# tomka/mitsuba-renderer

Measured on AMD Instinct MI355X. Metric: Msamples/s, higher is better.
Workload: dtype f32; 1 GPU; C3 1M-tri Cornell: 1024000-tri displaced walls TriMesh + 20480-tri dielectric icosphere + area light, path maxDepth=16 rrDepth=10, 1024x1024, ldsampler 64 spp per GPU (64 per frame, weak scaling), box filter; triangles=1044482, kd_nodes=551229, kd_indices=1101661, parallelism=ImageBlock tiles, morton(tx, ty) % 1 + one RCCL film reduce per frame

## Files before the change

include/mtsgpu.h:

```cpp
#ifndef MTSGPU_H
#define MTSGPU_H

#include <stdint.h>
#include <stddef.h>

#ifdef __cplusplus
extern "C" {
#endif

#define MTSGPU_ABI_VERSION 8

enum {
	MTSGPU_OK = 0,
	MTSGPU_EINVAL = -1,
	MTSGPU_EHIP = -2,
	MTSGPU_ENODEV = -3,
	MTSGPU_ECANCEL = -4,
	MTSGPU_ESTATE = -5
};

enum {
	MTSGPU_BSDF_LAMBERTIAN = 0,
	MTSGPU_BSDF_DIELECTRIC = 1,
	MTSGPU_BSDF_ROUGHMETAL = 2,
// ... 191 lines not shown
int  mtsgpu_bsdf_eval(mtsgpu_ctx *ctx, uint32_t bsdf_type, const float *params, int op, uint32_t n, const float *queries, float *out);
int  mtsgpu_bsdf_eval_table(mtsgpu_ctx *ctx, uint32_t n_bsdfs, const uint32_t *types, const float *params, uint32_t index, int op,
                            uint32_t n, const float *queries, float *out);
int  mtsgpu_sky_configure(const float *block, float *derived);
int  mtsgpu_lum_eval(mtsgpu_ctx *ctx, uint32_t lum_type, const float *block, int op, uint32_t n, const float *queries, float *out);
int  mtsgpu_scene_lum_eval(mtsgpu_ctx *ctx, int op, uint32_t n, const float *queries, float *out);
int  mtsgpu_vertex_color_eval(mtsgpu_ctx *ctx, uint32_t n, const uint32_t *prim, const float *uv, float *out);
int  mtsgpu_bsdf_eval_colored(mtsgpu_ctx *ctx, uint32_t bsdf_type, const float *params, uint32_t slots, const float color[3], int op,
                              uint32_t n, const float *queries, float *out);
int  mtsgpu_uv_texture_eval(mtsgpu_ctx *ctx, const mtsgpu_uv_texture *tex, uint32_t n, const uint32_t *prim, const float *rec, float *out);
int  mtsgpu_bsdf_eval_slots(mtsgpu_ctx *ctx, uint32_t bsdf_type, const float *params, const int32_t slot_source[2], const float color[3],
                            const float *values, int op, uint32_t n, const float *queries, float *out);
int  mtsgpu_shading_frame_eval(mtsgpu_ctx *ctx, uint32_t n, const uint32_t *prim, const float *rec, float *out);
int  mtsgpu_li_samples(mtsgpu_ctx *ctx, const uint32_t *pix_samples, uint32_t n, float *out);
int  mtsgpu_pass_samples(mtsgpu_ctx *ctx, uint32_t first, uint32_t n, float *out);

typedef struct mtsgpu_mesh {
	uint32_t n_verts, n_tris;
	const float    *positions;
	const float    *normals;
	const uint32_t *triangles;
	int32_t face_normals;
	int32_t bsdf;
	int32_t lum;
	int32_t shape_type;
	float   sphere_center[3];
	float   sphere_radius;
	int32_t sphere_inverted;
} mtsgpu_mesh;

// ... 58 lines not shown
```

mitsuba-renderer_amd/__init__.py:

```python
import ctypes as C
import os
import subprocess

import numpy as np

from . import abi, scenes, filmreduce, testmode
from .testmode import write_mfile, analyze

_HERE = os.path.dirname(os.path.abspath(__file__))
LIB_PATH = os.environ.get("MTSGPU_LIB") or os.path.join(_HERE, "libmtsgpu.so")

EXPORTS = [
    "mtsgpu_create", "mtsgpu_destroy", "mtsgpu_last_error", "mtsgpu_abi_version", "mtsgpu_source_hash", "mtsgpu_abi_sizeof", "mtsgpu_set_stream",
    "mtsgpu_upload_scene", "mtsgpu_set_camera", "mtsgpu_set_integrator", "mtsgpu_set_direct_integrator", "mtsgpu_set_sampler",
    "mtsgpu_set_tiles", "mtsgpu_set_rfilter", "mtsgpu_set_film_edges", "mtsgpu_tabulate_filter", "mtsgpu_set_film_buffer", "mtsgpu_set_options", "mtsgpu_render", "mtsgpu_sync",
    "mtsgpu_read_film", "mtsgpu_clear_film", "mtsgpu_get_stats", "mtsgpu_trace_rays", "mtsgpu_ld_tables",
    "mtsgpu_li_samples", "mtsgpu_flatten", "mtsgpu_flat_scene_get", "mtsgpu_flat_scene_free",
    "mtsgpu_flat_scene_kdstats", "mtsgpu_make_camera", "mtsgpu_make_camera_ortho", "mtsgpu_load_serialized", "mtsgpu_loaded_mesh_free",
    "mtsgpu_make_camera_crop", "mtsgpu_hbm_triad", "mtsgpu_sampler_values", "mtsgpu_random_values", "mtsgpu_set_tuning", "mtsgpu_gather_roof",
    "mtsgpu_create_multi", "mtsgpu_group_destroy", "mtsgpu_group_size", "mtsgpu_group_ctx", "mtsgpu_group_last_error",
    "mtsgpu_group_upload_scene", "mtsgpu_group_set_camera", "mtsgpu_group_set_integrator", "mtsgpu_group_set_sampler",
    "mtsgpu_group_set_rfilter", "mtsgpu_group_render", "mtsgpu_group_last_reduce_kind", "mtsgpu_group_rccl_ranks", "mtsgpu_group_reduce_note", "mtsgpu_bsdf_eval", "mtsgpu_bsdf_eval_table", "mtsgpu_replay_roof", "mtsgpu_group_set_tuning",
    "mtsgpu_sky_configure", "mtsgpu_lum_eval", "mtsgpu_scene_lum_eval", "mtsgpu_pass_samples",
    "mtsgpu_set_film_statistics", "mtsgpu_read_film_statistics", "mtsgpu_film_statistics_form", "mtsgpu_group_set_film_statistics",
    "mtsgpu_set_vertex_colors", "mtsgpu_group_set_vertex_colors", "mtsgpu_flat_scene_set_mesh_colors", "mtsgpu_flat_scene_vertex_colors",
    "mtsgpu_flat_scene_shape_has_colors", "mtsgpu_loaded_mesh_colors", "mtsgpu_vertex_color_eval", "mtsgpu_bsdf_eval_colored",
    "mtsgpu_set_uv_textures", "mtsgpu_group_set_uv_textures", "mtsgpu_flat_scene_set_mesh_texcoords", "mtsgpu_flat_scene_vertex_texcoords",
    "mtsgpu_flat_scene_shape_has_texcoords", "mtsgpu_loaded_mesh_texcoords", "mtsgpu_uv_texture_eval", "mtsgpu_bsdf_eval_slots",
    "mtsgpu_flatten_tangents", "mtsgpu_flat_scene_vertex_tangents", "mtsgpu_flat_scene_shape_has_tangents", "mtsgpu_upload_scene_tangents",
    "mtsgpu_group_upload_scene_tangents", "mtsgpu_shading_frame_eval",
]


class MtsGpuError(RuntimeError):
    pass


def load_serialized(path, shape_index=0, bsdf=-1, lum=-1, name=None):
    h = C.c_void_p(); m = abi.Mesh()
    rc = lib().mtsgpu_load_serialized(os.fsencode(path), int(shape_index), C.byref(h), C.byref(m))
    if rc != 0:
        raise MtsGpuError("mtsgpu_load_serialized: %s" % lib().mtsgpu_last_error(None).decode())
    try:
        pos = abi.np_from(m.positions, (m.n_verts, 3), np.float32)
        tri = abi.np_from(m.triangles, (m.n_tris, 3), np.uint32)
# ... 87 lines not shown
    L.mtsgpu_set_tiles.argtypes = [vp, C.c_int, C.c_int, C.c_int]
    L.mtsgpu_set_film_buffer.argtypes = [vp, vp]
    L.mtsgpu_set_rfilter.argtypes = [vp, C.c_float, C.c_float, f32p]
    L.mtsgpu_set_film_edges.argtypes = [vp, C.c_int]
    L.mtsgpu_tabulate_filter.argtypes = [C.c_int, C.c_float, C.c_float, C.c_float, f32p, f32p]
    L.mtsgpu_set_options.argtypes = [vp, C.c_uint64, C.c_int, C.c_int]
    L.mtsgpu_render.argtypes = [vp, C.POINTER(C.c_int)]
    L.mtsgpu_sync.argtypes = [vp]
    L.mtsgpu_read_film.argtypes = [vp, f32p]
    L.mtsgpu_clear_film.argtypes = [vp]
    L.mtsgpu_get_stats.argtypes = [vp, C.POINTER(abi.Stats)]
    L.mtsgpu_trace_rays.argtypes = [vp, f32p, C.c_uint32, C.c_int, u32p]
    L.mtsgpu_ld_tables.argtypes = [vp, C.c_uint32, f32p, f32p]
    L.mtsgpu_li_samples.argtypes = [vp, u32p, C.c_uint32, f32p]
    L.mtsgpu_pass_samples.argtypes = [vp, C.c_uint32, C.c_uint32, f32p]
    L.mtsgpu_flatten.argtypes = [C.POINTER(abi.SceneDesc), C.POINTER(abi.KdParams), C.POINTER(vp)]
    L.mtsgpu_flat_scene_get.argtypes = [vp]; L.mtsgpu_flat_scene_get.restype = C.POINTER(abi.Scene)
    L.mtsgpu_flat_scene_free.argtypes = [vp]; L.mtsgpu_flat_scene_free.restype = None
    L.mtsgpu_flat_scene_kdstats.argtypes = [vp, C.POINTER(C.c_double)]
    L.mtsgpu_make_camera.argtypes = [f32p, f32p, f32p, C.c_float, C.c_int, C.c_int, C.POINTER(abi.Camera)]
    L.mtsgpu_make_camera_ortho.argtypes = [f32p, f32p, f32p, C.c_float, C.c_float, C.c_int, C.c_int, C.POINTER(abi.Camera)]
    L.mtsgpu_load_serialized.argtypes = [C.c_char_p, C.c_int, C.POINTER(vp), C.POINTER(abi.Mesh)]
    L.mtsgpu_loaded_mesh_free.argtypes = [vp]; L.mtsgpu_loaded_mesh_free.restype = None
    L.mtsgpu_make_camera_crop.argtypes = [f32p, f32p, f32p, C.c_float] + [C.c_int] * 6 + [C.POINTER(abi.Camera)]
    L.mtsgpu_gather_roof.argtypes = [C.c_int, C.c_size_t, C.POINTER(C.c_double)]
    L.mtsgpu_set_tuning.argtypes = [vp, C.c_char_p, C.c_long]
    L.mtsgpu_sampler_values.argtypes = [vp, C.c_uint32, C.c_uint32, C.c_uint32, C.c_int, f32p]
    L.mtsgpu_random_values.argtypes = [vp, C.c_int, C.c_uint64, C.c_uint64, C.c_uint32, C.c_uint32, C.POINTER(C.c_uint64)]
    L.mtsgpu_bsdf_eval.argtypes = [vp, C.c_uint32, f32p, C.c_int, C.c_uint32, f32p, f32p]
    L.mtsgpu_bsdf_eval_table.argtypes = [vp, C.c_uint32, u32p, f32p, C.c_uint32, C.c_int, C.c_uint32, f32p, f32p]
# ... 300 lines not shown

    def sync(self):
        self._chk(lib().mtsgpu_sync(self._ctx), "sync")

    def film(self):
        cam = self.camera.c if hasattr(self.camera, "c") else self.camera
        out = np.zeros((cam.height, cam.width, 5), dtype=np.float32)
        self._chk(lib().mtsgpu_read_film(self._ctx, abi.ptr(out, abi.f32p)), "read_film")
        return out

    def stats(self):
        st = abi.Stats()
        self._chk(lib().mtsgpu_get_stats(self._ctx, C.byref(st)), "get_stats")
        return st.as_dict()

    def set_film_statistics(self, on=True):
        self._chk(lib().mtsgpu_set_film_statistics(self._ctx, int(bool(on))), "set_film_statistics")

    def film_statistics(self):
        cam = self.camera.c if hasattr(self.camera, "c") else self.camera
        var = np.zeros((cam.height, cam.width, 3), dtype=np.float32)
        n = np.zeros((cam.height, cam.width), dtype=np.uint32)
        self._chk(lib().mtsgpu_read_film_statistics(self._ctx, abi.ptr(var, abi.f32p), abi.ptr(n, abi.u32p)), "read_film_statistics")
        return var, n

    def film_statistics_form(self):
        return {0: "lane", 1: "wave"}.get(lib().mtsgpu_film_statistics_form(self._ctx))

    def trace_rays(self, rays, shadow=False):
        r = np.ascontiguousarray(rays, dtype=np.float32).reshape(-1, 8)
# ... 327 lines not shown
```

mitsuba-renderer_amd/csrc/api.cpp:

```cpp
#include "host.h"
#include "kernels.h"
#include "devmath.h"
#include "ctx.h"
#include <algorithm>
#include <cstdarg>
#include <cstdio>
#include <cstring>
#include <cstdlib>
#include <cmath>

using namespace mg;

namespace mg {
thread_local std::string g_lastError;

int fail(mtsgpu_ctx *ctx, int code, const char *fmt, ...) {
	char buf[512];
	va_list ap; va_start(ap, fmt); vsnprintf(buf, sizeof(buf), fmt, ap); va_end(ap);
	g_lastError = buf;
	if (ctx) ctx->error = buf;
	return code;
}
}

// ... 146 lines not shown
	cfg.weight_bsdf = 1 / (float) c->nBsdfSamples; cfg.weight_lum = 1 / (float) c->nLumSamples;
	cfg.frac_bsdf = c->nBsdfSamples / (float) (c->nLumSamples + c->nBsdfSamples);
	cfg.frac_lum = c->nLumSamples / (float) (c->nLumSamples + c->nBsdfSamples);
	cfg.sampler_kind = c->samplerKind;
	cfg.spp = effectiveSpp(c); cfg.ld_depth = c->ldDepth; cfg.seed = c->seed;
	cfg.strat_res = 1; while ((uint32_t) cfg.strat_res * (uint32_t) cfg.strat_res < cfg.spp) ++cfg.strat_res;
	cfg.slot_per_path = slotPerPath ? 1 : 0;
	cfg.ld_scr = c->ldScr; cfg.ld_perm = c->ldPerm; cfg.primes = c->primes;
	if (c->integrator == 1) {
		if (c->nLumSamples > 1) cfg.arr_size[cfg.arr_n++] = (uint32_t) c->nLumSamples;
		if (c->nBsdfSamples > 1) cfg.arr_size[cfg.arr_n++] = (uint32_t) c->nBsdfSamples;
		for (int a = 0; a < cfg.arr_n; ++a) { cfg.arr_off[a] = cfg.arr_total; cfg.arr_total += cfg.spp * cfg.arr_size[a]; }
	}
	cfg.arr_scr = c->arrScr; cfg.arr_perm = c->arrPerm; cfg.arr_pts = c->arrPts;
	cfg.filt_size_x = c->filtSizeX; cfg.filt_size_y = c->filtSizeY; cfg.filt_border = c->filtBorder; cfg.filt_values = c->filtValues;
	return cfg;
}

int ensureSampleArrays(mtsgpu_ctx *c, size_t nSlots, size_t nPaths) {
	if (c->integrator != 1 || (c->nLumSamples <= 1 && c->nBsdfSamples <= 1))
		return 0;
	if (c->samplerKind == MTSGPU_SAMPLER_HALTON || c->samplerKind == MTSGPU_SAMPLER_HAMMERSLEY)
		return fail(c, MTSGPU_EINVAL, "request2DArray() is not supported by QMC samplers! (halton.cpp:102-104, hammersley.cpp:112-114)");
	const uint32_t spp = effectiveSpp(c);
	size_t total = 0; int nArr = 0;
	for (int n : { c->nLumSamples, c->nBsdfSamples })
		if (n > 1) {
			if ((uint64_t) spp * (uint64_t) n > 65536ull)
				return fail(c, MTSGPU_EINVAL, "sampleCount x samples per strategy = %llu exceeds 65536 points per pixel", (unsigned long long) spp * n);
			total += (size_t) spp * n; ++nArr;
// ... 15 lines not shown
hipEvent_t *nextEventPair(mtsgpu_ctx *c, std::vector<std::pair<hipEvent_t, hipEvent_t>> &pool, size_t &used) {
	if (used == pool.size()) {
		hipEvent_t a, b;
		if (hipEventCreate(&a) != hipSuccess || hipEventCreate(&b) != hipSuccess) return nullptr;
		pool.emplace_back(a, b);
	}
	return &pool[used++].first;
}

long tuningOr(const mtsgpu_ctx *c, const char *key, long dflt);
void rayQueues(mtsgpu_ctx *c, const uint32_t *cur, const uint32_t *nxt) {
	const bool on = tuningOr(c, "ray_queues", 1) != 0;
	auto of = [&](const uint32_t *q, int k) -> float4 * { return !on || !q ? nullptr : (q == c->queueA ? c->rayqA[k] : (q == c->queueB ? c->rayqB[k] : nullptr)); };
	c->paths.rq_o = of(cur, 0); c->paths.rq_d = of(cur, 1); c->paths.rqn_o = of(nxt, 0); c->paths.rqn_d = of(nxt, 1);
}
struct RayQueuesOff { mtsgpu_ctx *c; ~RayQueuesOff() { rayQueues(c, nullptr, nullptr); c->q.nee_parked = 0; } };

hipEvent_t *nextTraceEvents(mtsgpu_ctx *c, int cls) {
	hipEvent_t *ev = nextEventPair(c, c->traceEvents, c->traceEvUsed);
	if (ev) {
		if (c->traceEvClass.size() < c->traceEvUsed) c->traceEvClass.resize(c->traceEvUsed);
		c->traceEvClass[c->traceEvUsed - 1] = (unsigned char) cls;
	}
	return ev;
}

int readCounters(mtsgpu_ctx *c) {
	HIPCHK(c, hipMemcpyAsync(c->hostCounters, c->q.counters, kNumCounters * kCounterStride * sizeof(uint32_t), hipMemcpyDeviceToHost, c->stream));
	HIPCHK(c, hipStreamSynchronize(c->stream));
	return 0;
}
// ... 13 lines not shown
		c->stats.trace_launches++;
		int rc = readCounters(c); if (rc) { c->q.force_static = 0; return rc; }
		c->q.force_static = 0;
		bool overflow = false;
		for (int b = 0; b < kNumBins; ++b) {
			uint32_t acc = 0;
			for (int k = 0; k < kBinShards; ++k) {
				views[b].prefix[k] = acc;
				const uint32_t cnt = c->hostCounters[(b * kBinShards + k) * kCounterStride];
				if (cnt > c->q.bin_seg_cap) overflow = true;
				acc += cnt;
			}
			views[b].prefix[kBinShards] = acc;
		}
		if (attempt == 0 && c->tuning.count("test_retry") && c->tuning["test_retry"]) overflow = true;
		if (!overflow) return 0;
		c->stats.bin_overflow_retries++;
	}
	return fail(c, MTSGPU_EHIP, "internal: bin segment overflow with static dealing");
}

int runDirectRounds(mtsgpu_ctx *c, const DConfig &cfg0, uint32_t nPaths, volatile const int *cancel) {
	hipStream_t s = c->stream;
	DConfig cfg = cfg0;
	const size_t counterBytes = kNumCounters * kCounterStride * sizeof(uint32_t);
	auto timedTrace = [&](int mode, bool bin, const uint32_t *queue, uint32_t n, bool coherent) -> int {
		hipEvent_t *ev = c->timeKernels ? nextTraceEvents(c, mode == 1 ? 2 : 0) : nullptr;
		if (ev) HIPCHK(c, hipEventRecord(ev[0], s));
		launch_trace(s, mode, c->countTraversal, bin, c->dsc, c->paths, c->q, queue, n, coherent);
		if (ev) HIPCHK(c, hipEventRecord(ev[1], s));
		HIPCHK(c, hipGetLastError());
// ... 66 lines not shown
	const int chunk = (int) tuningOr(c, "chunk", 8);
	uint32_t *cur = c->queueA, *nxt = c->queueB;
	uint32_t upper = nPaths;
	bool shadowPending = false;
	int b = 0;
	struct Restore {
		mtsgpu_ctx *c; hipStream_t s2; const bool &pending;
		~Restore() {
			if (pending) (void) hipStreamSynchronize(s2);
			c->q.dev_stats = nullptr; c->q.counters = c->counterSets; c->q.spill = c->spillClosest;
		}
	} restore{ c, s2, shadowPending };
	RayQueuesOff rqOff{ c };
	c->q.nee_parked = tuningOr(c, "nee_parked", 1) != 0 ? 1u : 0u;
	if (!c->q.nee_parked) { int rc = ensureNeeQueue(c); if (rc) return rc; }
	auto timed = [&](std::vector<std::pair<hipEvent_t, hipEvent_t>> &pool, size_t &used, hipStream_t s, int which, int cls = -1) -> int {
		if (!c->timeKernels) return 0;
		hipEvent_t *ev = which == 0 ? (cls >= 0 ? nextTraceEvents(c, cls) : nextEventPair(c, pool, used)) : &pool[used - 1].first;
		if (!ev) return fail(c, MTSGPU_EHIP, "hipEventCreate failed");
		HIPCHK(c, hipEventRecord(ev[which], s));
		return 0;
	};
	while (b < limit && upper > 0) {
		if (cancel && *cancel) return fail(c, MTSGPU_ECANCEL, "render cancelled");
		const int end = (int) std::min<long long>((long long) b + chunk, limit);
		for (; b < end; ++b) {
			uint32_t *set = counterSet(c, b), *prev = counterSet(c, b - 1);
			c->q.counters = set; c->q.next = nxt; c->q.spill = c->spillClosest;
			rayQueues(c, cur, nxt);
			int rc = timed(c->traceEvents, c->traceEvUsed, s1, 0, b == 0 ? 1 : 0); if (rc) return rc;
// ... 36 lines not shown
		upper = *hostNext;
	}
	if (shadowPending) {
		HIPCHK(c, hipStreamWaitEvent(s1, c->evShadow[(b - 1) & 1], 0));
		shadowPending = false;
	}
	return 0;
}

int collectDeviceStats(mtsgpu_ctx *c) {
	if (!c->devStatsUsed) return 0;
	c->devStatsUsed = false;
	unsigned long long h[kNumDevStats];
	HIPCHK(c, hipMemcpy(h, c->devStats, sizeof(h), hipMemcpyDeviceToHost));
	c->stats.rays_closest += h[kStatClosest]; c->stats.rays_shadow += h[kStatShadow]; c->stats.trace_launches += h[kStatLaunches];
	if (h[kStatOverflow]) return fail(c, MTSGPU_EHIP, "internal: bin segment overflow in a device-driven frame");
	return 0;
}

int runBounces(mtsgpu_ctx *c, const DConfig &cfg, uint32_t nPaths, volatile const int *cancel) {
	c->q.counters = c->counterSets; c->q.spill = c->spillClosest; c->q.dev_stats = nullptr;
	if (cfg.integrator == 1 && (cfg.n_lum > 1 || cfg.n_bsdf > 1))
		return runDirectRounds(c, cfg, nPaths, cancel);
	{
		const long sf = tuningOr(c, "sync_free", -1);
		if (sf == 1 || (sf < 0 && nPaths <= (8u << 20)))
			return runBouncesDevice(c, cfg, nPaths, cancel);
	}
	uint32_t nQ = nPaths;
	uint32_t *cur = c->queueA, *nxt = c->queueB;
	bool first = true;
	hipStream_t s = c->stream;
	const size_t setBytes = (size_t) kNumCounters * kCounterStride * sizeof(uint32_t);
	RayQueuesOff rqOff{ c };
	c->q.nee_parked = tuningOr(c, "nee_parked", 1) != 0 ? 1u : 0u;
	if (!c->q.nee_parked) { int rc = ensureNeeQueue(c); if (rc) return rc; }
	for (int b = 0; nQ > 0; ++b) {
		if (cancel && *cancel)
			return fail(c, MTSGPU_ECANCEL, "render cancelled");
		c->q.counters = counterSet(c, b); c->q.spill = c->spillClosest;
		HIPCHK(c, hipMemsetAsync(c->q.counters, 0, setBytes, s));
		c->q.next = nxt;
		rayQueues(c, cur, nxt);
		BinView views[kNumBins];
		int rc = traceAndBin(c, cur, nQ, first, views); if (rc) return rc;
		c->stats.rays_closest += nQ;
		hipEvent_t *sev = c->timeKernels ? nextEventPair(c, c->shadeEvents, c->shadeEvUsed) : nullptr;
		if (sev) HIPCHK(c, hipEventRecord(sev[0], s));
		for (int bin = 0; bin < kNumBins; ++bin)
			launch_shade(s, bin, c->dsc, c->paths, cfg, c->q, views[bin], nullptr, 0, nullptr, c->dcol, c->dtex, c->dtan);
		if (sev) HIPCHK(c, hipEventRecord(sev[1], s));
// ... 759 lines not shown
	tabulateFilter(kind, half_size, p0, p1, size_xy, values);
	return 0;
}

int mtsgpu_set_film_buffer(mtsgpu_ctx *c, void *device_ptr) {
	if (!c) return fail(nullptr, MTSGPU_EINVAL, "null context");
	if (c->ownFilm && c->film) (void) hipFree(c->film);
	c->film = (float *) device_ptr; c->ownFilm = false; c->filmPixels = 0;
	return 0;
}

int mtsgpu_set_tuning(mtsgpu_ctx *c, const char *key, long value) {
	if (!c || !key) return fail(c, MTSGPU_EINVAL, "null argument");
	struct Knob { const char *key; long lo, hi; };
	static const Knob knobs[] = { { "refill_min", 1, 64 }, { "desc_min", 1, 64 }, { "leaf_min", 1, 64 }, { "batch", 0, 64 },
	                              { "dyn_div", 0, 1 << 20 }, { "test_retry", 0, 1 }, { "sync_free", -1, 1 }, { "chunk", 1, 1024 }, { "blocks_per_cu", 0, (long) kTraceBlocksPerCuMax }, { "plain_below", 0, 1 << 30 }, { "dyn_min_rounds", 0, 1 << 20 }, { "shade_fused", 0, 1 }, { "ray_queues", 0, 1 }, { "nee_parked", 0, 1 }, { "stats_wave", -1, 1 } };
	for (const Knob &k : knobs)
		if (std::strcmp(k.key, key) == 0) {
			if (value < k.lo || value > k.hi) return fail(c, MTSGPU_EINVAL, "tuning knob %s: %ld outside [%ld, %ld]", key, value, k.lo, k.hi);
			c->tuning[key] = value;
			applyTuning(c);
			return 0;
		}
	return fail(c, MTSGPU_EINVAL, "unknown tuning knob '%s'", key);
}

int mtsgpu_set_options(mtsgpu_ctx *c, uint64_t max_paths, int count_traversal, int time_kernels) {
	if (!c) return fail(nullptr, MTSGPU_EINVAL, "null context");
	c->maxPaths = max_paths; c->countTraversal = count_traversal != 0; c->timeKernels = time_kernels != 0;
	return 0;
}
// ... 96 lines not shown
		for (int t = 0; t < tx * ty; ++t) {
			if (tileMorton((uint32_t) (t % tx), (uint32_t) (t / tx)) % (uint32_t) c->nParts != (uint32_t) c->part) continue;
			const int x0 = off + (t % tx) * bs, y0 = off + (t / tx) * bs;
			TileMeta tm{};
			tm.x0 = x0 + cx; tm.y0 = y0 + cy; tm.w = std::min(bs, off + RW - x0); tm.h = std::min(bs, off + RH - y0);
			tm.slot_base = (uint32_t) pixels.size(); tm.block_index = (uint32_t) tiles.size();
			tm.colour = (uint32_t) (((t % tx) & 1) + 2 * ((t / tx) & 1));
			tiles.push_back(tm);
			for (int y = tm.y0; y < tm.y0 + tm.h; ++y)
				for (int x = tm.x0; x < tm.x0 + tm.w; ++x)
					pixels.push_back((uint32_t) (y - off) * (uint32_t) keyW + (uint32_t) (x - off));
		}
		c->renderKey = key; c->renderListValid = false;
	}
	std::memset(&c->stats, 0, sizeof(c->stats));
	c->traceEvUsed = c->shadeEvUsed = 0;
	if (pixels.empty()) return 0;
	if (!reuse) {
		rc = ensureBuf(c, &c->pixelList, &c->pixelListCap, pixels.size()); if (rc) return rc;
		HIPCHK(c, hipMemcpyAsync(c->pixelList, pixels.data(), pixels.size() * sizeof(uint32_t), hipMemcpyHostToDevice, c->stream));
		HIPCHK(c, hipStreamSynchronize(c->stream));
		c->renderListValid = true;
	}

	const bool wideFilter = c->filtBorder > 0;
	if (wideFilter && 2 * c->filtBorder > bs) return fail(c, MTSGPU_EINVAL, "filter border %d too wide for block size %d", c->filtBorder, bs);
	const uint64_t maxPaths = c->maxPaths ? c->maxPaths : defaultMaxPaths(c);
	size_t slotsPerPass = (size_t) std::max<uint64_t>(1, std::min<uint64_t>(pixels.size(), maxPaths / spp));
	if (wideFilter) slotsPerPass = std::max<size_t>(slotsPerPass, (size_t) bs * bs);
	if ((uint64_t) slotsPerPass * spp > 0x7FFFFFFFull) return fail(c, MTSGPU_EINVAL, "pass too large");
// ... 178 lines not shown
	}
	if (kind == 2) {
		RR_CHK(hipMalloc((void **) &tmp, (size_t) n * 2 * sizeof(float4)));
		launch_gather_strided(s, tmp, c->paths.shq_o, n, stride); launch_gather_strided(s, tmp + n, c->paths.shq_d, n, stride);
		RR_CHK(hipMemcpyAsync(c->paths.shq_o, tmp, (size_t) n * sizeof(float4), hipMemcpyDeviceToDevice, s));
		RR_CHK(hipMemcpyAsync(c->paths.shq_d, tmp + n, (size_t) n * sizeof(float4), hipMemcpyDeviceToDevice, s));
		c->lastPass.shadowMax = 0;
	} else {
		launch_iota_strided(s, c->queueA, n, stride);
		launch_gather_strided(s, c->rayqA[0], c->paths.base + 0, n, stride * kPathSlots);
		launch_gather_strided(s, c->rayqA[1], c->paths.base + 1, n, stride * kPathSlots);
		rayQueues(c, c->queueA, nullptr);
	}
	RayQueuesOff rqOff{ c };
	c->q.nee_parked = mode == 1 ? 1u : 0u;
	const uint32_t *queue = mode == 1 ? c->q.shadow : c->queueA;
	RR_CHK(hipMemsetAsync(recLen, 0, (size_t) n * 4, s));
	RR_CHK(hipMemsetAsync(c->q.trace_counts, 0, kNumTraceCounts * sizeof(unsigned long long), s));
	RR_CHK(hipMemsetAsync(c->q.counters, 0, counterBytes, s));
	c->q.rec = rec; c->q.rec_len = recLen; c->q.rec_cap = cap;
	launch_trace(s, mode, true, bin, c->dsc, c->paths, c->q, queue, n, coherent);
	c->q.rec = c->q.rec_len = nullptr; c->q.rec_cap = 0;
	RR_CHK(hipGetLastError());
	std::vector<uint32_t> len(n);
	RR_CHK(hipMemcpyAsync(len.data(), recLen, (size_t) n * 4, hipMemcpyDeviceToHost, s));
	RR_CHK(hipStreamSynchronize(s));
	unsigned long long cnt[kNumTraceCounts];
	RR_CHK(hipMemcpy(cnt, c->q.trace_counts, sizeof(cnt), hipMemcpyDeviceToHost));
	std::vector<uint32_t> ord(n), first(cap + 2, 0u);
	unsigned long long total = 0, truncated = 0;
// ... 391 lines not shown
		launch_scene_lum_eval(c->stream, c->dsc, op, n, dQ, dOut);
		e = hipGetLastError();
	}
	if (e == hipSuccess) e = hipMemcpyAsync(out, dOut, (size_t) n * 16 * sizeof(float), hipMemcpyDeviceToHost, c->stream);
	if (e == hipSuccess) e = hipStreamSynchronize(c->stream);
	if (dQ) (void) hipFree(dQ);
	if (dOut) (void) hipFree(dOut);
	if (e != hipSuccess) return fail(c, MTSGPU_EHIP, "scene luminaire read-out failed: %s", hipGetErrorString(e));
	return 0;
}

int mtsgpu_li_samples(mtsgpu_ctx *c, const uint32_t *pix_samples, uint32_t n, float *out) {
	int rc = checkReady(c); if (rc) return rc;
	if (!pix_samples || !out) return fail(c, MTSGPU_EINVAL, "null argument");
	std::memset(&c->stats, 0, sizeof(c->stats));
	c->traceEvUsed = c->shadeEvUsed = 0;
	if (n == 0) return 0;
	const uint32_t spp = effectiveSpp(c);
	std::vector<uint32_t> keys(n);
	for (uint32_t i = 0; i < n; ++i) {
		const uint32_t x = pix_samples[3 * (size_t) i], y = pix_samples[3 * (size_t) i + 1], j = pix_samples[3 * (size_t) i + 2];
		if (x >= (uint32_t) c->cam.width || y >= (uint32_t) c->cam.height || j >= spp)
			return fail(c, MTSGPU_EINVAL, "sample %u: pixel or sample index out of range", i);
		keys[i] = (y + (uint32_t) c->cam.crop_offset_y) * (uint32_t) filmWidth(c) + x + (uint32_t) c->cam.crop_offset_x;
	}
	rc = ensurePaths(c, n); if (rc) return rc;
	rc = ensureBuf(c, &c->explicitSamples, &c->explicitCap, 3 * (size_t) n); if (rc) return rc;
	c->renderListValid = false; c->lastPass.valid = false;
	rc = ensureBuf(c, &c->pixelList, &c->pixelListCap, n); if (rc) return rc;
	HIPCHK(c, hipMemcpyAsync(c->explicitSamples, pix_samples, 3 * (size_t) n * sizeof(uint32_t), hipMemcpyHostToDevice, c->stream));
// ... 54 lines not shown
	HIPCHK(c, hipMemcpy2DAsync(misc.data(), 16, rec + 6, pitch, 16, n, hipMemcpyDeviceToHost, c->stream));
	HIPCHK(c, hipStreamSynchronize(c->stream));
	for (size_t i = 0; i < n; ++i) {
		uint32_t flags; int depth;
		std::memcpy(&flags, &Li[4 * i + 3], 4); std::memcpy(&depth, &thr[4 * i + 3], 4);
		float *o = out + 8 * i;
		const float4 L = settled_Li(make_float4(Li[4 * i], Li[4 * i + 1], Li[4 * i + 2], 0.0f),
		                            make_float4(parked[4 * i], parked[4 * i + 1], parked[4 * i + 2], parked[4 * i + 3]));
		o[0] = L.x; o[1] = L.y; o[2] = L.z; o[3] = (flags & F_ALPHA) ? 1.0f : 0.0f;
		o[4] = spos[4 * i]; o[5] = spos[4 * i + 1]; o[6] = (float) depth;
		std::memcpy(&o[7], &misc[4 * i + 3], 4);
	}
	return 0;
}

struct mtsgpu_flat_scene { FlatScene fs; };

int mtsgpu_flatten(const mtsgpu_scene_desc *desc, const mtsgpu_kd_params *kd, mtsgpu_flat_scene **out) {
	if (!desc || !out) return fail(nullptr, MTSGPU_EINVAL, "null argument");
	*out = nullptr;
	try {
		std::unique_ptr<mtsgpu_flat_scene> p(new mtsgpu_flat_scene());
		flattenScene(*desc, kd, p->fs);
		*out = p.release();
	} catch (const std::exception &e) {
		return fail(nullptr, MTSGPU_EINVAL, "%s", e.what());
	}
	return 0;
}

// ... 80 lines not shown
```

mitsuba-renderer_amd/csrc/ctx.h:

```cpp
#pragma once
#include "host.h"
#include "kernels.h"
#include <map>
#include <string>
#include <utility>
#include <vector>

struct mtsgpu_ctx {
	int device = 0;
	uint32_t nCUs = 256;
	hipStream_t stream = nullptr;
	bool ownStream = false;
	hipStream_t stream2 = nullptr;
	hipEvent_t evShade[2] = { nullptr, nullptr }, evShadow[2] = { nullptr, nullptr }, evCount = nullptr;
	std::string error;

	bool haveScene = false;
	mg::DScene dsc{};
	std::vector<void *> sceneAllocs;
	uint32_t nTris = 0;
	struct HostScene {
		uint32_t nVerts = 0;
		std::vector<uint32_t> triIdx, shapeTriOffset, shapeType, bsdfType, lumType;
		std::vector<int32_t> shapeBsdf;
// ... 43 lines not shown
	float4 *primSave = nullptr; size_t primSaveCap = 0;
	float4 *shqNee = nullptr; size_t shqNeeCap = 0;
	uint16_t *primes = nullptr;
	uint32_t *explicitSamples = nullptr; size_t explicitCap = 0;
	uint32_t *hostCounters = nullptr;
	uint32_t *counterSets = nullptr;
	uint32_t *spillClosest = nullptr, *spillShadow = nullptr;
	mg::BinView *viewsDev = nullptr;
	unsigned long long *devStats = nullptr;
	bool devStatsUsed = false;
	uint32_t binMask = 0x1FFu;
	unsigned long long *pathLen = nullptr;
	std::vector<void *> pathAllocs;

	mtsgpu_stats stats{};
	std::vector<std::pair<hipEvent_t, hipEvent_t>> traceEvents, shadeEvents;
	size_t traceEvUsed = 0, shadeEvUsed = 0;
	std::vector<unsigned char> traceEvClass;
	struct LastPass { bool valid = false; mg::DConfig cfg{}; size_t base = 0; uint32_t nSlots = 0, nPaths = 0, shadowMax = 0; } lastPass;
};


namespace mg {
extern thread_local std::string g_lastError;
int fail(mtsgpu_ctx *ctx, int code, const char *fmt, ...);
}

#define HIPCHK(ctx, expr) do { hipError_t e_ = (expr); if (e_ != hipSuccess) \
	return mg::fail(ctx, MTSGPU_EHIP, "%s failed: %s (%s:%d)", #expr, hipGetErrorString(e_), __FILE__, __LINE__); } while (0)
```

mitsuba-renderer_amd/csrc/kernels.h:

```cpp
#pragma once
#include <hip/hip_runtime.h>
#include <stdint.h>

namespace mg {

constexpr int kNumBsdfTypes = 10;
constexpr int kNumBins = kNumBsdfTypes + 1;
#ifndef MG_TRACE_BLOCK
#define MG_TRACE_BLOCK 512
#endif
constexpr int kTraceBlock = MG_TRACE_BLOCK;
static_assert(kTraceBlock % 256 == 0 && kTraceBlock <= 1024, "whole multiples of four waves");
#ifdef MG_TRACE_WGS
constexpr unsigned trace_blocks_per_cu(int) { return MG_TRACE_WGS; }
#else
constexpr unsigned trace_blocks_per_cu(int mode) { return (mode == 0 ? 24u : 32u) / (kTraceBlock / 64); }
#endif
constexpr unsigned trace_waves_per_simd(int mode) { return trace_blocks_per_cu(mode) * (kTraceBlock / 64) / 4; }
constexpr unsigned kTraceBlocksPerCuMax = 2048 / kTraceBlock;
#ifndef MG_STACK_LDS
#define MG_STACK_LDS 10
#endif
#ifndef MG_TOP_PAIRS
#define MG_TOP_PAIRS (MG_TRACE_BLOCK >= 512 ? 1024 : 128)
// ... 13 lines not shown
constexpr int kCounterStride = 32;
constexpr int kBsdfNParams = 16;
constexpr int kBinShards = 16;
constexpr uint32_t kShadeAllBins = ((1u << kNumBins) - 1u) & ~(1u << 9);
constexpr int kNumCounters = kNumBins * kBinShards + 4;
constexpr int kCounterSets = 2;
constexpr int kCntNext = kNumBins * kBinShards, kCntShadow = kCntNext + 1, kCntDynClosest = kCntNext + 2, kCntDynShadow = kCntNext + 3;
constexpr int kNextWord = kCntNext * kCounterStride, kShadowWord = kCntShadow * kCounterStride;
#ifndef MG_SHADE_BLOCK
#define MG_SHADE_BLOCK 1024
#endif
constexpr int kShadeBlock = MG_SHADE_BLOCK;
constexpr int kNumTraceCounts = 16;
enum { kCntPairGlobal = 8, kCntPairLds = 9, kCntNodeGlobal = 10, kCntNodeLds = 11, kCntTail = 12, kCntSpill = 13, kCntHead = 14 };
enum : uint32_t { kReqPair = 1, kReqNode = 2, kReqLeaf = 3, kReqRay = 4, kReqHit = 5, kReqNone = 0xFFFFFFFFu };
enum { kStatClosest = 0, kStatShadow = 1, kStatOverflow = 2, kStatLaunches = 3, kNumDevStats = 4 };

struct DScene {
	const uint2    *nodes;
	const uint4    *leaf_ta;
	const float4   *tri_pos;
	const float4   *tri_nrm;
	const int32_t  *shape_bsdf, *shape_lum;
	const uint32_t *shape_bin;
	const uint32_t *shape_type;
	const float    *shape_params;
	const float    *env_pixels, *env_pdf, *env_cdf;
	uint32_t        env_width, env_height, env_pdf_width, env_pdf_height;
	uint32_t        has_shapes;
	const uint32_t *shape_flags, *shape_tri_offset;
	const uint32_t *bsdf_type;
// ... 95 lines not shown
	uint32_t arr_size[2], arr_off[2], arr_total;
	const uint32_t *arr_scr;
	const uint16_t *arr_perm;
	const float2 *arr_pts;
	int32_t sampler_kind;
	uint32_t spp; int32_t ld_depth;
	int32_t strat_res;
	uint64_t seed;
	int32_t slot_per_path;
	float filt_size_x, filt_size_y;
	int32_t filt_border;
	const float *filt_values;
	const uint32_t *ld_scr;
	const uint16_t *ld_perm;
	const uint16_t *primes;
};

struct DQueues {
	uint32_t *bins_base;
	uint32_t bin_stride;
	uint32_t bin_seg_cap;
	uint4 *bin_hits;
	__host__ __device__ uint32_t *bin(int b) const { return bins_base + (size_t) b * bin_stride; }
	uint32_t *next;
	uint32_t *shadow;
	uint32_t *counters;
	unsigned long long *trace_counts;
	uint32_t *rec, *rec_len;
	uint32_t rec_cap;
	unsigned long long *dev_stats;
	uint32_t *spill;
	uint32_t spill_stride;
	uint32_t desc_min;
	uint32_t leaf_min;
	uint32_t refill_min;
	uint32_t coherent;
	uint32_t n_cus;
	uint32_t force_static;
	uint32_t tune_batch;
	uint32_t tune_dyn_div;
	uint32_t tune_refill;
	uint32_t tune_plain_below;
	uint32_t tune_dyn_min_rounds;
	uint32_t tune_blocks_per_cu;
// ... 109 lines not shown
```

mitsuba-renderer_amd/csrc/shade_path.h:

```cpp
#pragma once
#include "shade_bsdf.h"

namespace mg {

#ifndef MG_SHADE_PACKED
#define MG_SHADE_PACKED 0
#endif
constexpr int kRowStride = MG_SHADE_PACKED ? kPathSlots : kPathSlots + 1;
struct ShadeRow {
	float4 *base; uint32_t x;
	__device__ __forceinline__ float4 &operator[](int k) const { return base[MG_SHADE_PACKED ? ((uint32_t) k ^ x) : (uint32_t) k]; }
};
__device__ __forceinline__ uint32_t shade_row_index(uint32_t lane, uint32_t k) { return lane * kRowStride + (MG_SHADE_PACKED ? (k ^ (lane & 7u)) : k); }

template <int BT, bool ROUNDS, bool SKY, int VCOL, bool TAN = false>
__device__ __forceinline__ void shade_path(const DScene &sc, const DPaths &ps, const DConfig &cfg, const uint32_t id,
                                           const float4 ro, const float4 rd, const uint4 h, const float4 T4, const float4 L4,
                                           const ShadeRow row, bool &continues, bool &wantShadow, V3 &neeV, V3 &shO, V3 &shD, const DColors &col,
                                           const DTextures &tex, const DTangents &tan = DTangents{ nullptr, nullptr }) {
	{
		const int mode = ROUNDS ? cfg.dr_mode : 0;
		const bool skipToNee = ROUNDS && mode == 1 && cfg.dr_index > 0, skipToBsdf = ROUNDS && mode == 2;
		const V3 rayO(ro.x, ro.y, ro.z), rayD(rd.x, rd.y, rd.z);
		const bool valid = h.w != kNoPrim;
		V3 thr(T4.x, T4.y, T4.z), Li(L4.x, L4.y, L4.z);
		int depth = __float_as_int(T4.w);
		uint32_t flags = __float_as_uint(L4.w);
		PathSampler smp;
		uint2 misc_zw;
		{
			const uint4 r = reinterpret_cast<const uint4 &>(row[6]);
			smp.stream = (uint64_t) r.x | ((uint64_t) r.y << 32);
			smp.slot = cfg.slot_per_path ? id : (id / cfg.spp);
			smp.j = r.z;
			misc_zw = make_uint2(r.z, r.w);
			smp.d1 = (flags >> F_D1_SHIFT) & 0xFFu; smp.d2 = (flags >> F_D2_SHIFT) & 0xFFu;
		}
		const bool direct = cfg.integrator == 1;
		Its its;
		if (valid) {
			if (TAN) fill_its_tan(sc, tan, rayO, rayD, __uint_as_float(h.x), h.w, __uint_as_float(h.y), __uint_as_float(h.z), row[0], row[1], row[3], its);
			else fill_its(sc, rayO, rayD, __uint_as_float(h.x), h.w, __uint_as_float(h.y), __uint_as_float(h.z), row[0], row[1], row[3], its);
		}
		const int shapeLum = valid ? sc.shape_lum[its.shape] : -1;

		do {
			if (skipToNee || skipToBsdf) {
			} else if (flags & F_FIRST) {
				flags &= ~F_FIRST;
				if (valid) flags |= F_ALPHA;
				if (!direct && !(depth <= cfg.max_depth || cfg.max_depth < 0))
					break;
			} else {
// ... 5 lines not shown
				V3 lvalue(0, 0, 0), lp(0, 0, 0), ln(0, 0, 0);
				int llum = -1;
				if (valid) {
					if (shapeLum >= 0) {
						const float *LP = sc.lum_params + kLumStride * (size_t) shapeLum;
						lp = its.p; ln = its.geoN; llum = shapeLum;
						lvalue = (dot(-rayD, its.geoN) <= 0) ? V3(0, 0, 0) : V3(LP[0], LP[1], LP[2]);
						hitLuminaire = true;
					}
				} else {
					if (sc.background_lum >= 0) {
						llum = sc.background_lum;
						lvalue = background_le<SKY>(sc, rayD);
						hitLuminaire = true;
					} else {
						if (!direct) depth++;
						break;
					}
				}
				if (hitLuminaire) {
					const float lumPdf = (!(sampledType & T_DELTA)) ? pdf_luminaire(sc, rayO, llum, lp, ln, -rayD) : 0.0f;
					const float weight = direct ? mi_weight(bsdfPdf * cfg.frac_bsdf, lumPdf * cfg.frac_lum) * cfg.weight_bsdf
					                            : mi_weight(bsdfPdf, lumPdf);
					Li.x += thr.x * lvalue.x * bsdfVal.x * weight;
					Li.y += thr.y * lvalue.y * bsdfVal.y * weight;
					Li.z += thr.z * lvalue.z * bsdfVal.z * weight;
				}
				if (!valid || direct)
					break;
				flags &= ~F_EMITTED;
				if (depth >= cfg.rr_depth && !(sampledType & T_TRANSMISSION)) {
					const float approxAlbedo = smin(0.9f, smax(smax(bsdfVal.x, bsdfVal.y), bsdfVal.z));
					if (sampler_next1d(cfg, smp) > approxAlbedo)
						break;
					thr = thr * (1.0f / approxAlbedo);
				}
				thr = thr * bsdfVal;
				depth++;
				if (!(depth <= cfg.max_depth || cfg.max_depth < 0))
					break;
			}

			if (!valid) {
				if (skipToNee || skipToBsdf) break;
				if ((flags & F_EMITTED) && sc.background_lum >= 0) {
					const V3 le = background_le<SKY>(sc, rayD);
					Li.x += thr.x * le.x; Li.y += thr.y * le.y; Li.z += thr.z * le.z;
				}
				break;
			}
			if (BT == kNumBsdfTypes)
				break;
			const int bsdfIdx = sc.shape_bsdf[its.shape];
// ... 86 lines not shown
			const V3 wo(its.shS.x * woL.x + its.shT.x * woL.y + its.shN.x * woL.z,
			            its.shS.y * woL.x + its.shT.y * woL.y + its.shN.y * woL.z,
			            its.shS.z * woL.x + its.shT.z * woL.y + its.shN.z * woL.z);
			const float woDotGeoN = dot(its.geoN, wo);
			if (woDotGeoN * woL.z <= 0 && strict)
				break;
			row[0] = make_float4(its.p.x, its.p.y, its.p.z, kEpsilon);
			row[1] = make_float4(wo.x, wo.y, wo.z, MG_INF);
			row[5] = make_float4(bsdfVal.x, bsdfVal.y, bsdfVal.z, bsdfPdf);
			flags = (flags & 0x00FFFFFFu) | (sampledType << F_ST_SHIFT);
			continues = true;
		} while (false);
		if (!continues) { row[0] = ro; row[1] = rd; }

		flags = (flags & ~((0xFFu << F_D1_SHIFT) | (0xFFu << F_D2_SHIFT))) | (smp.d1 << F_D1_SHIFT) | (smp.d2 << F_D2_SHIFT);
		row[3] = make_float4(thr.x, thr.y, thr.z, __int_as_float(depth));
		row[4] = make_float4(Li.x, Li.y, Li.z, __uint_as_float(flags));
		reinterpret_cast<uint4 &>(row[6]) = make_uint4((uint32_t) (smp.stream & 0xFFFFFFFFull), (uint32_t) (smp.stream >> 32), misc_zw.x, misc_zw.y);
	}

}

#ifndef MG_SHADE_WAVES
#define MG_SHADE_WAVES 0
#endif
#if MG_SHADE_WAVES
#define MG_SHADE_BOUNDS __launch_bounds__(kShadeBlock, MG_SHADE_WAVES)
#else
#define MG_SHADE_BOUNDS __launch_bounds__(kShadeBlock)
#endif
struct ShadeShared {
// ... 193 lines not shown
```

mitsuba-renderer_amd/csrc/trace.hip:

```cpp
#include "kdevice.h"

namespace mg {


__device__ __forceinline__ uint32_t lanes_below(uint64_t mask) {
	return __builtin_amdgcn_mbcnt_hi((uint32_t) (mask >> 32), __builtin_amdgcn_mbcnt_lo((uint32_t) mask, 0u));
}
size_t trace_spill_levels() { return kSpillLevels; }
size_t trace_stack_levels() { return kStackLDS + kSpillLevels; }
uint32_t trace_top_nodes() { return kTopNodes; }

__device__ __forceinline__ const uint4 *leaf_head(const DTraceScene &sc, uint32_t e) { return &sc.leaf_ta[kLeafStride * (size_t) e]; }
__device__ __forceinline__ const uint4 *leaf_tail(const DTraceScene &sc, uint32_t e, uint32_t half) { return &sc.leaf_ta[kLeafStride * (size_t) e + 1 + half]; }

template <int MODE, bool COUNT, bool BIN, bool PARKED>
__device__ __forceinline__ void trace_body(const DTraceScene &sc, const DPaths &ps, const DQueues &q, const TracePlan &plan,
                                           const uint32_t *queue, uint32_t n, const uint32_t first, const uint32_t stride,
                                           uint32_t (*s_stack)[kTraceBlock], uint32_t (*s_mbox)[kTraceBlock], const uint4 *s_top) {
	uint32_t g_pair = 0, l_pair = 0, g_node = 0, l_node = 0, g_tail = 0, g_spill = 0, g_head = 0;
	uint32_t rec_n = 0, rec_slot = 0;
	auto rec_add = [&](uint32_t kind, uint32_t idx) {
		if (COUNT && q.rec) {
			if (rec_n < q.rec_cap) q.rec[(size_t) rec_slot * q.rec_cap + rec_n] = (kind << 29) | idx;
			rec_n++;
// ... 56 lines not shown
				if (base < n) { sup_base = (uint32_t) base; sup_left = (n - sup_base < B) ? n - sup_base : B; }
				else dyn_done = true;
			}
		}
		const uint32_t remaining = sup_left;
		if (nlive == 0u || (remaining != 0u && wantRays)) {
			if (MODE == 0) {
				int bin = -1;
				constexpr bool hitsToBins = BIN;
				if (done) {
					if (!hitsToBins) st_stream<1>(&ps.hit(id), make_uint4(__float_as_uint(best_t), __float_as_uint(best_u), __float_as_uint(best_v), best_prim));
					if (BIN) {
						bin = kNumBins - 1;
						if (found) {
							bin = (int) sc.shape_bin[best_shape];
						}
					}
				}
				if (BIN) {
					uint32_t cnt = 0, rank = 0;
					#pragma unroll
					for (int b = 0; b < kNumBins; ++b) {
						const uint64_t m = __builtin_amdgcn_ballot_w64(bin == b);
						if (lane == (uint32_t) b) cnt = (uint32_t) __popcll(m);
						if (bin == b) rank = lanes_below(m);
					}
					uint32_t base = 0;
					if (lane < (uint32_t) kNumBins && cnt != 0u)
						base = atomicAdd(&q.counters[(lane * kBinShards + shard) * kCounterStride], cnt);
					base = __shfl(base, bin < 0 ? 0 : bin);
// ... 278 lines not shown
	if (t < (uint32_t) (kNumBins * kBinShards)) {
		const uint32_t c = cur[t * kCounterStride];
		s_cnt[t] = c;
		if (c > bin_seg_cap && dev_stats) atomicAdd(&dev_stats[kStatOverflow], 1ull);
	}
	if (t < (uint32_t) kNumCounters) next_set[t * kCounterStride] = 0u;
	__syncthreads();
	if (t < (uint32_t) kNumBins) {
		uint32_t acc = 0;
		for (int k = 0; k < kBinShards; ++k) {
			views[t].prefix[k] = acc;
			const uint32_t c = s_cnt[t * kBinShards + k];
			acc += c < bin_seg_cap ? c : bin_seg_cap;
		}
		views[t].prefix[kBinShards] = acc;
	}
}

template <int MODE, bool COUNT, bool BIN, bool PARKED = false>
static void launch_trace_t(hipStream_t s, const DScene &sc, const DPaths &ps, const DQueues &q, const uint32_t *queue, uint32_t n,
                           const uint32_t *n_dev) {
	unsigned blocks = trace_plan(n, MODE, q).blocks;
	if (n_dev) {
		const unsigned minBatch = (q.tune_batch >= 1 && q.tune_batch <= 64) ? q.tune_batch : (q.coherent ? 64u : 8u);
		unsigned perCu = trace_blocks_per_cu(MODE);
		if (q.tune_blocks_per_cu && q.tune_blocks_per_cu < perCu) perCu = q.tune_blocks_per_cu;
		blocks = std::min<unsigned>(blocks_for(n, minBatch * (kTraceBlock / 64)), q.n_cus * perCu);
	}
	if (!blocks) return;
	hipLaunchKernelGGL((k_trace<MODE, COUNT, BIN, PARKED>), dim3(blocks), dim3(kTraceBlock), 0, s, trace_scene(sc), ps, q, queue, n, n_dev);
// ... 27 lines not shown
```

Measured before the change: 306.0 Msamples/s.

## Drop missed rays from shading bins when there is no background emitter

When the scene has no background luminaire, closest-hit rays that miss are no longer written to the miss bin. They are treated as finished, so no shading thread is spent on them. To keep the depth and Russian-roulette semantics unchanged, the shader defers the depth increment and adds it back when it writes the path state. The change also adds per-bin entry counters exposed through a new API call, which costs a few device atomics per frame.

```diff
diff --git a/include/mtsgpu.h b/include/mtsgpu.h
--- a/include/mtsgpu.h
+++ b/include/mtsgpu.h
@@ -229,6 +229,7 @@
 int  mtsgpu_shading_frame_eval(mtsgpu_ctx *ctx, uint32_t n, const uint32_t *prim, const float *rec, float *out);
 int  mtsgpu_li_samples(mtsgpu_ctx *ctx, const uint32_t *pix_samples, uint32_t n, float *out);
 int  mtsgpu_pass_samples(mtsgpu_ctx *ctx, uint32_t first, uint32_t n, float *out);
+int  mtsgpu_bin_entries(mtsgpu_ctx *ctx, uint64_t *out);
 
 typedef struct mtsgpu_mesh {
 	uint32_t n_verts, n_tris;
diff --git a/mitsuba-renderer_amd/__init__.py b/mitsuba-renderer_amd/__init__.py
--- a/mitsuba-renderer_amd/__init__.py
+++ b/mitsuba-renderer_amd/__init__.py
@@ -28,7 +28,7 @@
     "mtsgpu_set_uv_textures", "mtsgpu_group_set_uv_textures", "mtsgpu_flat_scene_set_mesh_texcoords", "mtsgpu_flat_scene_vertex_texcoords",
     "mtsgpu_flat_scene_shape_has_texcoords", "mtsgpu_loaded_mesh_texcoords", "mtsgpu_uv_texture_eval", "mtsgpu_bsdf_eval_slots",
     "mtsgpu_flatten_tangents", "mtsgpu_flat_scene_vertex_tangents", "mtsgpu_flat_scene_shape_has_tangents", "mtsgpu_upload_scene_tangents",
-    "mtsgpu_group_upload_scene_tangents", "mtsgpu_shading_frame_eval",
+    "mtsgpu_group_upload_scene_tangents", "mtsgpu_shading_frame_eval", "mtsgpu_bin_entries",
 ]
 
 
@@ -146,6 +146,7 @@
     L.mtsgpu_ld_tables.argtypes = [vp, C.c_uint32, f32p, f32p]
     L.mtsgpu_li_samples.argtypes = [vp, u32p, C.c_uint32, f32p]
     L.mtsgpu_pass_samples.argtypes = [vp, C.c_uint32, C.c_uint32, f32p]
+    L.mtsgpu_bin_entries.argtypes = [vp, C.POINTER(C.c_uint64)]
     L.mtsgpu_flatten.argtypes = [C.POINTER(abi.SceneDesc), C.POINTER(abi.KdParams), C.POINTER(vp)]
     L.mtsgpu_flat_scene_get.argtypes = [vp]; L.mtsgpu_flat_scene_get.restype = C.POINTER(abi.Scene)
     L.mtsgpu_flat_scene_free.argtypes = [vp]; L.mtsgpu_flat_scene_free.restype = None
@@ -476,6 +477,11 @@
         self._chk(lib().mtsgpu_get_stats(self._ctx, C.byref(st)), "get_stats")
         return st.as_dict()
 
+    def bin_entries(self):
+        out = (C.c_uint64 * (abi.BSDF_NTYPES + 1))()
+        self._chk(lib().mtsgpu_bin_entries(self._ctx, out), "bin_entries")
+        return [int(v) for v in out]
+
     def set_film_statistics(self, on=True):
         self._chk(lib().mtsgpu_set_film_statistics(self._ctx, int(bool(on))), "set_film_statistics")
 
diff --git a/mitsuba-renderer_amd/csrc/api.cpp b/mitsuba-renderer_amd/csrc/api.cpp
--- a/mitsuba-renderer_amd/csrc/api.cpp
+++ b/mitsuba-renderer_amd/csrc/api.cpp
@@ -184,6 +184,11 @@
 	}
 	cfg.arr_scr = c->arrScr; cfg.arr_perm = c->arrPerm; cfg.arr_pts = c->arrPts;
 	cfg.filt_size_x = c->filtSizeX; cfg.filt_size_y = c->filtSizeY; cfg.filt_border = c->filtBorder; cfg.filt_values = c->filtValues;
+	{
+		const auto it = c->tuning.find("miss_shaded");
+		const bool rounds = c->integrator == 1 && (c->nLumSamples > 1 || c->nBsdfSamples > 1);
+		cfg.miss_settled = (c->dsc.background_lum < 0 && !rounds && !(it != c->tuning.end() && it->second == 1)) ? 1 : 0;
+	}
 	return cfg;
 }
 
@@ -229,7 +234,7 @@
 	auto of = [&](const uint32_t *q, int k) -> float4 * { return !on || !q ? nullptr : (q == c->queueA ? c->rayqA[k] : (q == c->queueB ? c->rayqB[k] : nullptr)); };
 	c->paths.rq_o = of(cur, 0); c->paths.rq_d = of(cur, 1); c->paths.rqn_o = of(nxt, 0); c->paths.rqn_d = of(nxt, 1);
 }
-struct RayQueuesOff { mtsgpu_ctx *c; ~RayQueuesOff() { rayQueues(c, nullptr, nullptr); c->q.nee_parked = 0; } };
+struct RayQueuesOff { mtsgpu_ctx *c; ~RayQueuesOff() { rayQueues(c, nullptr, nullptr); c->q.nee_parked = 0; c->q.miss_settled = 0; } };
 
 hipEvent_t *nextTraceEvents(mtsgpu_ctx *c, int cls) {
 	hipEvent_t *ev = nextEventPair(c, c->traceEvents, c->traceEvUsed);
@@ -273,7 +278,10 @@
 			views[b].prefix[kBinShards] = acc;
 		}
 		if (attempt == 0 && c->tuning.count("test_retry") && c->tuning["test_retry"]) overflow = true;
-		if (!overflow) return 0;
+		if (!overflow) {
+			for (int b = 0; b < kNumBins; ++b) c->binEntries[b] += views[b].prefix[kBinShards];
+			return 0;
+		}
 		c->stats.bin_overflow_retries++;
 	}
 	return fail(c, MTSGPU_EHIP, "internal: bin segment overflow with static dealing");
@@ -370,6 +378,7 @@
 	RayQueuesOff rqOff{ c };
 	c->q.nee_parked = tuningOr(c, "nee_parked", 1) != 0 ? 1u : 0u;
 	if (!c->q.nee_parked) { int rc = ensureNeeQueue(c); if (rc) return rc; }
+	c->q.miss_settled = cfg.miss_settled ? 1u : 0u;
 	auto timed = [&](std::vector<std::pair<hipEvent_t, hipEvent_t>> &pool, size_t &used, hipStream_t s, int which, int cls = -1) -> int {
 		if (!c->timeKernels) return 0;
 		hipEvent_t *ev = which == 0 ? (cls >= 0 ? nextTraceEvents(c, cls) : nextEventPair(c, pool, used)) : &pool[used - 1].first;
@@ -436,6 +445,7 @@
 	unsigned long long h[kNumDevStats];
 	HIPCHK(c, hipMemcpy(h, c->devStats, sizeof(h), hipMemcpyDeviceToHost));
 	c->stats.rays_closest += h[kStatClosest]; c->stats.rays_shadow += h[kStatShadow]; c->stats.trace_launches += h[kStatLaunches];
+	for (int b = 0; b < kNumBins; ++b) c->binEntries[b] += h[kStatBin0 + b];
 	if (h[kStatOverflow]) return fail(c, MTSGPU_EHIP, "internal: bin segment overflow in a device-driven frame");
 	return 0;
 }
@@ -457,6 +467,7 @@
 	RayQueuesOff rqOff{ c };
 	c->q.nee_parked = tuningOr(c, "nee_parked", 1) != 0 ? 1u : 0u;
 	if (!c->q.nee_parked) { int rc = ensureNeeQueue(c); if (rc) return rc; }
+	c->q.miss_settled = cfg.miss_settled ? 1u : 0u;
 	for (int b = 0; nQ > 0; ++b) {
 		if (cancel && *cancel)
 			return fail(c, MTSGPU_ECANCEL, "render cancelled");
@@ -1246,7 +1257,7 @@
 	if (!c || !key) return fail(c, MTSGPU_EINVAL, "null argument");
 	struct Knob { const char *key; long lo, hi; };
 	static const Knob knobs[] = { { "refill_min", 1, 64 }, { "desc_min", 1, 64 }, { "leaf_min", 1, 64 }, { "batch", 0, 64 },
-	                              { "dyn_div", 0, 1 << 20 }, { "test_retry", 0, 1 }, { "sync_free", -1, 1 }, { "chunk", 1, 1024 }, { "blocks_per_cu", 0, (long) kTraceBlocksPerCuMax }, { "plain_below", 0, 1 << 30 }, { "dyn_min_rounds", 0, 1 << 20 }, { "shade_fused", 0, 1 }, { "ray_queues", 0, 1 }, { "nee_parked", 0, 1 }, { "stats_wave", -1, 1 } };
+	                              { "dyn_div", 0, 1 << 20 }, { "test_retry", 0, 1 }, { "sync_free", -1, 1 }, { "chunk", 1, 1024 }, { "blocks_per_cu", 0, (long) kTraceBlocksPerCuMax }, { "plain_below", 0, 1 << 30 }, { "dyn_min_rounds", 0, 1 << 20 }, { "shade_fused", 0, 1 }, { "ray_queues", 0, 1 }, { "nee_parked", 0, 1 }, { "stats_wave", -1, 1 }, { "miss_shaded", 0, 1 } };
 	for (const Knob &k : knobs)
 		if (std::strcmp(k.key, key) == 0) {
 			if (value < k.lo || value > k.hi) return fail(c, MTSGPU_EINVAL, "tuning knob %s: %ld outside [%ld, %ld]", key, value, k.lo, k.hi);
@@ -1373,6 +1384,7 @@
 		c->renderKey = key; c->renderListValid = false;
 	}
 	std::memset(&c->stats, 0, sizeof(c->stats));
+	std::memset(c->binEntries, 0, sizeof(c->binEntries));
 	c->traceEvUsed = c->shadeEvUsed = 0;
 	if (pixels.empty()) return 0;
 	if (!reuse) {
@@ -1581,6 +1593,7 @@
 	}
 	RayQueuesOff rqOff{ c };
 	c->q.nee_parked = mode == 1 ? 1u : 0u;
+	c->q.miss_settled = 0;
 	const uint32_t *queue = mode == 1 ? c->q.shadow : c->queueA;
 	RR_CHK(hipMemsetAsync(recLen, 0, (size_t) n * 4, s));
 	RR_CHK(hipMemsetAsync(c->q.trace_counts, 0, kNumTraceCounts * sizeof(unsigned long long), s));
@@ -2002,6 +2015,7 @@
 	int rc = checkReady(c); if (rc) return rc;
 	if (!pix_samples || !out) return fail(c, MTSGPU_EINVAL, "null argument");
 	std::memset(&c->stats, 0, sizeof(c->stats));
+	std::memset(c->binEntries, 0, sizeof(c->binEntries));
 	c->traceEvUsed = c->shadeEvUsed = 0;
 	if (n == 0) return 0;
 	const uint32_t spp = effectiveSpp(c);
@@ -2086,6 +2100,12 @@
 	return 0;
 }
 
+int mtsgpu_bin_entries(mtsgpu_ctx *c, uint64_t *out) {
+	if (!c || !out) return fail(c, MTSGPU_EINVAL, "null argument");
+	for (int b = 0; b < kNumBins; ++b) out[b] = c->binEntries[b];
+	return 0;
+}
+
 struct mtsgpu_flat_scene { FlatScene fs; };
 
 int mtsgpu_flatten(const mtsgpu_scene_desc *desc, const mtsgpu_kd_params *kd, mtsgpu_flat_scene **out) {
diff --git a/mitsuba-renderer_amd/csrc/ctx.h b/mitsuba-renderer_amd/csrc/ctx.h
--- a/mitsuba-renderer_amd/csrc/ctx.h
+++ b/mitsuba-renderer_amd/csrc/ctx.h
@@ -81,6 +81,7 @@
 	std::vector<void *> pathAllocs;
 
 	mtsgpu_stats stats{};
+	uint64_t binEntries[mg::kNumBins] = {};
 	std::vector<std::pair<hipEvent_t, hipEvent_t>> traceEvents, shadeEvents;
 	size_t traceEvUsed = 0, shadeEvUsed = 0;
 	std::vector<unsigned char> traceEvClass;
diff --git a/mitsuba-renderer_amd/csrc/kernels.h b/mitsuba-renderer_amd/csrc/kernels.h
--- a/mitsuba-renderer_amd/csrc/kernels.h
+++ b/mitsuba-renderer_amd/csrc/kernels.h
@@ -51,7 +51,7 @@
 constexpr int kNumTraceCounts = 16;
 enum { kCntPairGlobal = 8, kCntPairLds = 9, kCntNodeGlobal = 10, kCntNodeLds = 11, kCntTail = 12, kCntSpill = 13, kCntHead = 14 };
 enum : uint32_t { kReqPair = 1, kReqNode = 2, kReqLeaf = 3, kReqRay = 4, kReqHit = 5, kReqNone = 0xFFFFFFFFu };
-enum { kStatClosest = 0, kStatShadow = 1, kStatOverflow = 2, kStatLaunches = 3, kNumDevStats = 4 };
+enum { kStatClosest = 0, kStatShadow = 1, kStatOverflow = 2, kStatLaunches = 3, kStatBin0 = 4, kNumDevStats = kStatBin0 + kNumBins };
 
 struct DScene {
 	const uint2    *nodes;
@@ -177,6 +177,7 @@
 	const uint32_t *ld_scr;
 	const uint16_t *ld_perm;
 	const uint16_t *primes;
+	int32_t miss_settled;
 };
 
 struct DQueues {
@@ -191,6 +192,7 @@
 	unsigned long long *trace_counts;
 	uint32_t *rec, *rec_len;
 	uint32_t rec_cap;
+	uint32_t miss_settled;
 	unsigned long long *dev_stats;
 	uint32_t *spill;
 	uint32_t spill_stride;
diff --git a/mitsuba-renderer_amd/csrc/shade_path.h b/mitsuba-renderer_amd/csrc/shade_path.h
--- a/mitsuba-renderer_amd/csrc/shade_path.h
+++ b/mitsuba-renderer_amd/csrc/shade_path.h
@@ -37,6 +37,7 @@
 			smp.d1 = (flags >> F_D1_SHIFT) & 0xFFu; smp.d2 = (flags >> F_D2_SHIFT) & 0xFFu;
 		}
 		const bool direct = cfg.integrator == 1;
+		const bool settled = !ROUNDS && cfg.miss_settled && !direct;
 		Its its;
 		if (valid) {
 			if (TAN) fill_its_tan(sc, tan, rayO, rayD, __uint_as_float(h.x), h.w, __uint_as_float(h.y), __uint_as_float(h.z), row[0], row[1], row[3], its);
@@ -72,7 +73,7 @@
 						lvalue = background_le<SKY>(sc, rayD);
 						hitLuminaire = true;
 					} else {
-						if (!direct) depth++;
+						if (!direct && !settled) depth++;
 						break;
 					}
 				}
@@ -87,14 +88,16 @@
 				if (!valid || direct)
 					break;
 				flags &= ~F_EMITTED;
-				if (depth >= cfg.rr_depth && !(sampledType & T_TRANSMISSION)) {
+				if (depth >= cfg.rr_depth + (settled ? 1 : 0) && !(sampledType & T_TRANSMISSION)) {
 					const float approxAlbedo = smin(0.9f, smax(smax(bsdfVal.x, bsdfVal.y), bsdfVal.z));
-					if (sampler_next1d(cfg, smp) > approxAlbedo)
+					if (sampler_next1d(cfg, smp) > approxAlbedo) {
+						if (settled) depth--;
 						break;
+					}
 					thr = thr * (1.0f / approxAlbedo);
 				}
 				thr = thr * bsdfVal;
-				depth++;
+				if (!settled) depth++;
 				if (!(depth <= cfg.max_depth || cfg.max_depth < 0))
 					break;
 			}
@@ -211,7 +214,7 @@
 		if (!continues) { row[0] = ro; row[1] = rd; }
 
 		flags = (flags & ~((0xFFu << F_D1_SHIFT) | (0xFFu << F_D2_SHIFT))) | (smp.d1 << F_D1_SHIFT) | (smp.d2 << F_D2_SHIFT);
-		row[3] = make_float4(thr.x, thr.y, thr.z, __int_as_float(depth));
+		row[3] = make_float4(thr.x, thr.y, thr.z, __int_as_float(depth + ((settled && continues) ? 1 : 0)));
 		row[4] = make_float4(Li.x, Li.y, Li.z, __uint_as_float(flags));
 		reinterpret_cast<uint4 &>(row[6]) = make_uint4((uint32_t) (smp.stream & 0xFFFFFFFFull), (uint32_t) (smp.stream >> 32), misc_zw.x, misc_zw.y);
 	}
diff --git a/mitsuba-renderer_amd/csrc/trace.hip b/mitsuba-renderer_amd/csrc/trace.hip
--- a/mitsuba-renderer_amd/csrc/trace.hip
+++ b/mitsuba-renderer_amd/csrc/trace.hip
@@ -94,6 +94,8 @@
 						bin = kNumBins - 1;
 						if (found) {
 							bin = (int) sc.shape_bin[best_shape];
+						} else if (q.miss_settled) {
+							bin = -1;
 						}
 					}
 				}
@@ -402,6 +404,7 @@
 			acc += c < bin_seg_cap ? c : bin_seg_cap;
 		}
 		views[t].prefix[kBinShards] = acc;
+		if (dev_stats && acc) atomicAdd(&dev_stats[kStatBin0 + t], (unsigned long long) acc);
 	}
 }
 
```

Result: faster. 310.2 Msamples/s (median of 6 runs) (+1.4%).
